# mprib/caliscope

Hardware: NVIDIA H100
Metric: lm_iterations_per_sec (higher is better)
Workload: dtype f64

## Files before the change

### caliscope_b200/csrc/cb_engine.cu

```cuda
#include <cuda_runtime.h>
#include <dlfcn.h>
#if defined(__x86_64__)
#include <emmintrin.h>
#endif
#include <nvtx3/nvToolsExt.h>

#include <algorithm>
#include <atomic>
#include <chrono>
#include <cmath>
#include <limits>
#include <cstdio>
#include <cstdlib>
#include <cstring>
#include <condition_variable>
#include <cub/cub.cuh>
#include <deque>
#include <functional>
#include <map>
#include <memory>
#include <mutex>
#include <string>
#include <thread>
#include <type_traits>
// ... 509 lines not shown
    k.trial_reduce = cb::trial_reduce_kernel<S>;
    k.schur_finalize = cb::schur_finalize_kernel<S>;
    k.schur_finalize_peer = cb::schur_finalize_peer_kernel<S>;
    with_bool(held.cams(), [&](auto hc) {
      constexpr bool HC = decltype(hc)::value;
      k.reduced_prep = cb::reduced_prep_kernel<S, HC>;
      k.small_rig_step = cb::small_rig_step_kernel<S, HC>;
    });
    k.comp_build = cb::comp_build_kernel<S>;
    k.cov_point = cb::cov_point_kernel<S>;
    with_lanes(pt_lanes, [&](auto lanes) {
      constexpr int L = decltype(lanes)::value;
      k.pt_stage_bytes = cb::pt_stage_bytes<S, L>();
      with_bool(cam_in_smem, [&](auto sm) {
        constexpr bool SM = decltype(sm)::value;
        with_bool(!held.fixp.empty(), [&](auto fp) {
          k.pt_backsub = cb::pt_backsub_kernel<S, L, SM, decltype(fp)::value>;
        });
        with_bool(held.points(), [&](auto hp) {
          constexpr bool HP = decltype(hp)::value;
          with_bool(dups, [&](auto d) {
            constexpr bool D = decltype(d)::value;
            k.pt_pass = cb::pt_pass_kernel<S, L, D, SM, false, HP>;
            k.pt_pass_cov = cb::pt_pass_kernel<S, L, D, SM, true, HP>;
          });
        });
      });
    });
    if (pcg_mode != 2) k.pcg = cb::pcg_cluster_kernel<1, S, 1>;
    else
      k.pcg = pcg_cl == 2 ? cb::pcg_cluster_kernel<2, S, 2> : pcg_cl == 6 ? cb::pcg_cluster_kernel<2, S, 6>
            : pcg_cl == 12 ? cb::pcg_cluster_kernel<2, S, 12> : cb::pcg_cluster_kernel<2, S, 18>;
  });
  return k;
}

struct CbBaProblem {
  int device = 0, num_sms = 132;
  int n_cams = 0, n_pts = 0, P = 6, nP = 0, n_obs = 0, n_params = 0;
  int LD = 0, n_blk = 0, n_tiles = 0, n_split = 1, k_chunks = 0, K_pad = 0;
  int n_chunks = 0, pt_grid = 0, pt_lanes = 32, n_dups = 0;
  int cam_in_smem = 0;
  size_t pt_smem = 0, bs_smem = 0;
  Kernels k;
  std::vector<int> h_cam_off;
  std::vector<int> h_perm, h_slot;
  std::vector<int> h_iflags;
  bool order_auto = false, order_identity = true;
  int ncp = 0;
  int *d_cam_xoff = nullptr, *d_cam_slot = nullptr, *d_klist = nullptr;
  bool schur_sparse = false;
  double schur_flop_issued = 0.0;
  std::vector<void*> allocs;
  int* d_cam_flags = nullptr;
  double* d_cam_const = nullptr;
  double2 *d_cm_xy = nullptr, *d_pm_xy = nullptr;
  int *d_cm_pt = nullptr, *d_cm_orig = nullptr, *d_cam_start = nullptr;
  int *d_chunk_cam = nullptr, *d_chunk_begin = nullptr, *d_chunk_end = nullptr, *d_cam_chunk_start = nullptr;
  int *d_pt_start = nullptr, *d_pm_orig = nullptr, *d_pm_cam = nullptr, *d_pm_pt = nullptr;
  const int *d_obs_cam = nullptr, *d_obs_pt = nullptr;
  const double* d_obs_xy = nullptr;
  std::vector<int> h_cam_flags;
  std::vector<double> h_cam_const;
  int *d_tile_of = nullptr, *d_tile_slot_start = nullptr, *d_tile_slots = nullptr;
  cb::SyItem* d_items = nullptr;
  int n_items = 0, n_slots = 0;
  CUtensorMap zt_map{};
  unsigned char* d_active = nullptr;
  HeldSet held;
  double *d_lo = nullptr, *d_hi = nullptr;
  int bounds_for = -1;
  double *d_x = nullptr, *d_xc[2] = {nullptr, nullptr}, *d_xp4[2] = {nullptr, nullptr};
  double *d_camtab[2] = {nullptr, nullptr}, *d_Upk[2] = {nullptr, nullptr}, *d_gc[2] = {nullptr, nullptr},
         *d_costsum[2] = {nullptr, nullptr};
  double *d_partial = nullptr, *d_camcost = nullptr, *d_V6 = nullptr, *d_gp = nullptr, *d_Dp2 = nullptr,
         *d_Dc2 = nullptr, *d_Linv6 = nullptr, *d_tvec = nullptr, *d_Zt = nullptr, *d_part = nullptr,
         *d_tpart = nullptr, *d_red = nullptr, *d_Minv = nullptr, *d_dc = nullptr, *d_dp = nullptr,
         *d_bpart = nullptr, *d_sc = nullptr, *d_red2 = nullptr, *d_out2 = nullptr;
  unsigned long long* d_gmax = nullptr;
  unsigned int* d_counter = nullptr;
  cb::LmState* d_state = nullptr;
  cb::LmState* h_state = nullptr;
  cb::LmLogRow* d_log = nullptr;
  int log_cap = 4096;
  cudaEvent_t ev0 = nullptr, ev1 = nullptr, ev2 = nullptr, ev3 = nullptr, ev_state[2] = {nullptr, nullptr};
  cudaEvent_t ev_pp[2][4] = {{nullptr, nullptr, nullptr, nullptr}, {nullptr, nullptr, nullptr, nullptr}};
  cudaStream_t cap_stream = nullptr;
  TrialGraph trial_graph;
  TrialGraph loop_graph;
  int pcg_cs = 1, pcg_rows = 0, pcg_mode = 2, pcg_cl = 1, pcg_npa = 0;
  bool direct_solve = false;
  size_t direct_smem = 0;
  size_t pcg_smem = 0;
  int n_c = 0, n_comp = 0, n_dim_max = 0, n_cblk = 0;
  cb::ConstraintTables ct = {};
  double *d_c_rs[2] = {nullptr, nullptr}, *d_c_dirw[2] = {nullptr, nullptr}, *d_compL = nullptr, *d_gpt = nullptr;
  int* d_pt_comp = nullptr;
  size_t comp_build_smem = 0, comp_back_smem = 0;
  std::vector<int> h_ga, h_gb;
  std::vector<double> h_cdist, h_cw;
  int red_slots = 64;
  CbPeerGroup* peer = nullptr;
  int cov_n = 0;
  double *d_covA = nullptr, *d_covC = nullptr, *d_covD = nullptr, *d_covS = nullptr, *d_covDiag = nullptr,
         *d_covR = nullptr, *d_covPt = nullptr;
  int *d_covRank = nullptr, *d_covFail = nullptr;
  unsigned char* d_covFree = nullptr;
  float cov_ms[3] = {0.f, 0.f, 0.f};
  double solve_host_us[4] = {0.0, 0.0, 0.0, 0.0};
  size_t red_len() const { return (size_t)nP * nP + 3 * (size_t)nP + 1 + red_slots; }
  cb::CPtr2 c_camtab() const { return {{d_camtab[0], d_camtab[1]}}; }
  cb::Ptr2 m_camtab() const { return {{d_camtab[0], d_camtab[1]}}; }
  cb::CPtr2 c_xp() const { return {{d_xp4[0], d_xp4[1]}}; }
  cb::Ptr2 m_xp() const { return {{d_xp4[0], d_xp4[1]}}; }
  cb::Ptr2 m_xc() const { return {{d_xc[0], d_xc[1]}}; }
  cb::CPtr2 c_Upk() const { return {{d_Upk[0], d_Upk[1]}}; }
  cb::Ptr2 m_Upk() const { return {{d_Upk[0], d_Upk[1]}}; }
  cb::CPtr2 c_gc() const { return {{d_gc[0], d_gc[1]}}; }
  cb::Ptr2 m_gc() const { return {{d_gc[0], d_gc[1]}}; }
  cb::CPtr2 c_costsum() const { return {{d_costsum[0], d_costsum[1]}}; }
  cb::Ptr2 m_costsum() const { return {{d_costsum[0], d_costsum[1]}}; }
  cb::CPtr2 c_crs() const { return {{d_c_rs[0], d_c_rs[1]}}; }
  cb::Ptr2 m_crs() const { return {{d_c_rs[0], d_c_rs[1]}}; }
  cb::CPtr2 c_cdirw() const { return {{d_c_dirw[0], d_c_dirw[1]}}; }
  cb::Ptr2 m_cdirw() const { return {{d_c_dirw[0], d_c_dirw[1]}}; }
};

namespace {

template <typename T>
int palloc(CbBaProblem* p, T** ptr, size_t n) {
  CB_TRY(dalloc(ptr, n));
  p->allocs.push_back((void*)*ptr);
  return CB_OK;
}

int bits_for(unsigned long long v) {
  int b = 1;
  while (b < 64 && (v >> b) != 0ull) ++b;
  return b;
}

void destroy_graph(TrialGraph& g) {
  if (g.exec) cudaGraphExecDestroy(g.exec);
  if (g.graph) cudaGraphDestroy(g.graph);
  g.exec = nullptr; g.graph = nullptr; g.valid = false; g.n_kernels = 0;
}

cudaStream_t side_stream() {
  thread_local std::map<int, cudaStream_t> streams;
  int dev = 0;
  cudaGetDevice(&dev);
  auto it = streams.find(dev);
  if (it != streams.end()) return it->second;
  cudaStream_t s = nullptr;
  cudaStreamCreateWithFlags(&s, cudaStreamNonBlocking);
  streams[dev] = s;
  return s;
}

int choose_camera_order(CbBaProblem* p, const int* cam_order, cudaStream_t st) {
  const int nc = p->n_cams;
  p->h_perm.resize(nc); p->h_slot.resize(nc);
  for (int i = 0; i < nc; ++i) p->h_perm[i] = i;
  p->order_auto = false;
  if (cam_order) {
    std::vector<char> seen(nc, 0);
    for (int i = 0; i < nc; ++i) {
      const int c = cam_order[i];
      if (c < 0 || c >= nc || seen[c]) { g_last_error = "cam_order is not a permutation of 0..n_cams-1"; return CB_E_INVALID; }
      seen[c] = 1;
      p->h_perm[i] = c;
    }
  } else {
    const int cams_per_tile = std::max(1, cb::SY_TILE / p->P);
    const double avg = (double)p->n_obs / std::max(p->n_pts, 1);
    if (p->n_blk >= 3 && avg <= nc / 3.0) {
      p->order_auto = true;
      const int stride = std::max(1, p->n_pts / 8192), ns = cdiv(p->n_pts, stride);
      unsigned int* d_W;
      ScopedFree sf(st);
      CB_TRY(sf.alloc(&d_W, (size_t)nc * nc));
      CB_CUDA(cudaMemsetAsync(d_W, 0, sizeof(unsigned int) * nc * nc, st));
      CB_LAUNCH(cb::covis_kernel, cdiv((long long)ns * 32, 256), 256, 0, st, p->d_pt_start, p->d_pm_cam, p->n_pts, stride, nc, d_W);
      std::vector<unsigned int> W((size_t)nc * nc);
      CB_CUDA(cudaMemcpyAsync(W.data(), d_W, sizeof(unsigned int) * nc * nc, cudaMemcpyDeviceToHost, st));
      CB_CUDA(cudaStreamSynchronize(st));
      std::vector<char> placed(nc, 0);
      std::vector<int> order;
      int start = 0;
      unsigned long long best = ~0ull;
      for (int c = 0; c < nc; ++c) {
        unsigned long long tot = 0;
        for (int q = 0; q < nc; ++q) if (q != c) tot += W[(size_t)c * nc + q];
        if (tot < best) { best = tot; start = c; }
      }
      order.push_back(start); placed[start] = 1;
      while ((int)order.size() < nc) {
        int pick = -1;
        unsigned long long bw = 0;
        const int lo = std::max(0, (int)order.size() - cams_per_tile);
        for (int c = 0; c < nc; ++c) {
          if (placed[c]) continue;
          unsigned long long w = 0;
          for (int k = lo; k < (int)order.size(); ++k) w += W[(size_t)c * nc + order[k]];
          if (pick < 0 || w > bw) { pick = c; bw = w; }
        }
        order.push_back(pick); placed[pick] = 1;
      }
      auto off_mass = [&](const std::vector<int>& ord) {
        std::vector<int> tile(nc);
        for (int i = 0; i < nc; ++i) tile[ord[i]] = (i * p->P) / cb::SY_TILE;
        unsigned long long m = 0;
        for (int a = 0; a < nc; ++a)
          for (int b = 0; b < nc; ++b)
            if (tile[a] != tile[b]) m += W[(size_t)a * nc + b];
        return m;
      };
      std::vector<int> ident(nc);
      for (int i = 0; i < nc; ++i) ident[i] = i;
      if (off_mass(order) < 0.8 * off_mass(ident)) p->h_perm = order;
    }
  }
  p->order_identity = true;
  for (int i = 0; i < nc; ++i) {
    p->h_slot[p->h_perm[i]] = i;
    if (p->h_perm[i] != i) p->order_identity = false;
  }
  CB_CUDA(cudaMemcpyAsync(p->d_cam_slot, p->h_slot.data(), sizeof(int) * nc, cudaMemcpyHostToDevice, st));
  return CB_OK;
}

struct XyUpload {
  bool started = false;
  std::atomic<int> finished{0};
  cudaEvent_t ev = nullptr;
  int rc = CB_OK;
  std::string err;
  ScopedFree pinned;
  void join() {
    if (!started) return;
    while (!finished.load(std::memory_order_acquire)) std::this_thread::yield();
    started = false;
  }
  int wait(cudaStream_t st) {
    join();
    if (rc != CB_OK) { g_last_error = err; return rc; }
    if (ev) CB_CUDA(cudaStreamWaitEvent(st, ev, 0));
    return CB_OK;
  }
  ~XyUpload() {
    join();
    if (ev) { cudaEventSynchronize(ev); cudaEventDestroy(ev); }
  }
};

int build_indices(CbBaProblem* p, const int* d_obs_cam, const int* d_obs_pt, const double* d_obs_xy,
                  const int* cam_order, cudaStream_t st, XyUpload* xy_upload) {
  const int n = p->n_obs;
  const int TB = 256, G = cdiv(std::max(n, 1), TB);
  ScopedFree sf(st);
  int* d_bad;
  CB_TRY(sf.alloc(&d_bad, 2));
  CB_CUDA(cudaMemsetAsync(d_bad, 0, 2 * sizeof(int), st));
  CB_LAUNCH(cb::validate_kernel, G, TB, 0, st, d_obs_cam, d_obs_pt, n, p->n_cams, p->n_pts, d_bad);

  unsigned long long *k_in, *k_out;
  int *v_in, *v_out, *pm_pt, *pm_cam, *cm_cam;
  CB_TRY(sf.alloc(&k_in, n));
  CB_TRY(sf.alloc(&k_out, n));
  CB_TRY(sf.alloc(&v_in, n));
  CB_TRY(sf.alloc(&v_out, n));
  CB_TRY(sf.alloc(&cm_cam, n));
  pm_pt = p->d_pm_pt; pm_cam = p->d_pm_cam;

  CB_LAUNCH(cb::make_keys_kernel, G, TB, 0, st, d_obs_pt, d_obs_cam, (long long)p->n_cams, n, k_in, v_in);
  const int kb = bits_for((unsigned long long)p->n_pts * (unsigned long long)p->n_cams);
  CB_CUB(sf, cub::DeviceRadixSort::SortPairs, k_in, k_out, v_in, p->d_pm_orig, n, 0, kb, st);
  g_launches.fetch_add(4);
  CB_LAUNCH(cb::split_keys_kernel, G, TB, 0, st, k_out, (long long)p->n_cams, n, pm_pt, pm_cam);
  CB_LAUNCH(cb::lower_bound_kernel, cdiv(p->n_pts + 1, TB), TB, 0, st, pm_pt, n, p->n_pts, p->d_pt_start);
  CB_LAUNCH(cb::count_dups_kernel, G, TB, 0, st, pm_pt, pm_cam, n, d_bad + 1);
  CB_TRY(choose_camera_order(p, cam_order, st));
  if (!p->order_identity) CB_LAUNCH(cb::remap_kernel, G, TB, 0, st, pm_cam, (const int*)p->d_cam_slot, n);
  CB_LAUNCH(cb::make_keys_kernel, G, TB, 0, st, pm_cam, pm_pt, (long long)p->n_pts, n, k_in, v_in);
  CB_CUB(sf, cub::DeviceRadixSort::SortPairs, k_in, k_out, v_in, v_out, n, 0, kb, st);
  g_launches.fetch_add(4);
  CB_LAUNCH(cb::split_keys_kernel, G, TB, 0, st, k_out, (long long)p->n_pts, n, cm_cam, v_in);
  CB_LAUNCH(cb::lower_bound_kernel, cdiv(p->n_cams + 1, TB), TB, 0, st, cm_cam, n, p->n_cams, p->d_cam_start);
  if (xy_upload) CB_TRY(xy_upload->wait(st));
  CB_LAUNCH(cb::cm_gather_kernel, G, TB, 0, st, v_out, p->d_pm_orig, pm_pt,
            reinterpret_cast<const double2*>(d_obs_xy), n, p->d_cm_pt, p->d_cm_orig, p->d_cm_xy);
  CB_LAUNCH(cb::pm_gather_kernel, G, TB, 0, st, p->d_pm_orig, reinterpret_cast<const double2*>(d_obs_xy), n, p->d_pm_xy);
  std::vector<int> cam_start(p->n_cams + 1);
  int bad[2] = {0, 0};
  CB_CUDA(cudaMemcpyAsync(cam_start.data(), p->d_cam_start, sizeof(int) * (p->n_cams + 1), cudaMemcpyDeviceToHost, st));
  CB_CUDA(cudaMemcpyAsync(bad, d_bad, 2 * sizeof(int), cudaMemcpyDeviceToHost, st));
  CB_CUDA(cudaStreamSynchronize(st));
  if (bad[0]) {
    g_last_error = "obs_cam / obs_pt index out of range in " + std::to_string(bad[0]) + " observations";
    return CB_E_INVALID;
  }
  p->n_dups = bad[1];
  std::vector<int> cc, cbeg, cend, ccs(p->n_cams + 1);
  const int chunk = cb::RJ_CHUNK;
  for (int c = 0; c < p->n_cams; ++c) {
    ccs[c] = (int)cc.size();
    for (int b = cam_start[c]; b < cam_start[c + 1]; b += chunk) {
      cc.push_back(c);
      cbeg.push_back(b);
      cend.push_back(std::min(b + chunk, cam_start[c + 1]));
    }
  }
  ccs[p->n_cams] = (int)cc.size();
  p->n_chunks = (int)cc.size();
  CB_TRY(palloc(p, &p->d_chunk_cam, cc.size()));
  CB_TRY(palloc(p, &p->d_chunk_begin, cc.size()));
  CB_TRY(palloc(p, &p->d_chunk_end, cc.size()));
  if (!cc.empty()) {
    CB_CUDA(cudaMemcpyAsync(p->d_chunk_cam, cc.data(), sizeof(int) * cc.size(), cudaMemcpyHostToDevice, st));
    CB_CUDA(cudaMemcpyAsync(p->d_chunk_begin, cbeg.data(), sizeof(int) * cc.size(), cudaMemcpyHostToDevice, st));
    CB_CUDA(cudaMemcpyAsync(p->d_chunk_end, cend.data(), sizeof(int) * cc.size(), cudaMemcpyHostToDevice, st));
  }
  CB_CUDA(cudaMemcpyAsync(p->d_cam_chunk_start, ccs.data(), sizeof(int) * ccs.size(), cudaMemcpyHostToDevice, st));
  CB_CUDA(cudaStreamSynchronize(st));
  return CB_OK;
}

int run_cam_prep(CbBaProblem* p, const double* xc, double* camtab, cudaStream_t st) {
  CB_LAUNCH(cb::cam_prep_kernel, cdiv(p->n_cams, 64), 64, 0, st, xc, p->d_cam_flags, p->d_cam_const, p->n_cams, p->P, camtab);
  return CB_OK;
}

void launch_resjac(CbBaProblem* p, int mode, const cb::LmState* st_dev, int flip, int loss, double fscale, double* out2,
                   cudaStream_t st) {
  if (p->n_chunks == 0) return;
  CB_LAUNCH(p->k.resjac[mode], p->n_chunks, cb::RJ_THREADS, 0, st, st_dev, flip, p->d_chunk_cam,
            p->d_chunk_begin, p->d_chunk_end, p->d_cm_xy, p->d_cm_pt, p->d_cm_orig, p->c_camtab(), p->c_xp(), loss,
            fscale, p->d_partial, out2);
}

void launch_pt_pass(CbBaProblem* p, bool cov, cudaStream_t st) {
  const auto pt_pass = cov ? p->k.pt_pass_cov : p->k.pt_pass;
  CB_LAUNCH(pt_pass, p->pt_grid, cb::PT_WARPS * 32, p->pt_smem, st, p->d_state,
            p->d_pt_start, p->d_pm_cam, p->d_pm_xy, p->d_pt_comp, p->n_pts, p->n_cams, p->c_camtab(), p->c_xp(),
            p->d_V6, p->d_gp, p->d_Dp2, cov ? p->d_covR : p->d_Linv6, p->d_tvec, p->d_Zt, (size_t)p->LD, p->d_gmax,
            cov ? p->d_covRank : nullptr, p->held.ppri);
}

void launch_pt_backsub(CbBaProblem* p, double* dp_out, cudaStream_t st) {
  const int bstride = p->pt_grid + p->n_comp;
  CB_LAUNCH(p->k.pt_backsub, p->pt_grid, cb::PT_WARPS * 32, p->bs_smem, st, p->d_state,
            p->d_pt_start, p->d_pm_cam, p->d_pm_xy, p->d_pt_comp, p->n_pts, p->n_cams, p->nP, p->c_camtab(),
            p->m_xp(), p->d_dc, p->d_Linv6, p->d_tvec, p->d_gp, p->d_Dp2, dp_out, p->d_bpart, bstride);
}

int launch_pcg(CbBaProblem* p, const cb::LmState* st_dev, double tol2, int max_iter, cudaStream_t st) {
  const ClusterConfig c(p->pcg_cs, cb::PCG_THREADS, p->pcg_cs, p->pcg_smem, st);
  const double* S = p->d_red;
  const double* b = p->d_red + (size_t)p->nP * p->nP;
  CB_CUDA(cudaLaunchKernelEx(&c.cfg, p->k.pcg, st_dev, S, b, (const double*)p->d_Minv, p->nP, p->pcg_npa, p->pcg_rows,
                             tol2, max_iter, p->d_dc, p->d_sc));
  g_launches.fetch_add(1);
  return CB_OK;
}

int camera_pass(CbBaProblem* p, int flip, int mode, cudaStream_t st) {
  const int loss = 0;
  const double fscale = 1.0;
  launch_resjac(p, 0, p->d_state, flip, loss, fscale, nullptr, st);
  if (p->n_c)
    CB_LAUNCH((cb::constraint_eval_kernel<false>), p->n_cblk, cb::CC_THREADS, 0, st, (const cb::LmState*)p->d_state, flip,
              p->ct, p->c_xp(), loss, fscale, p->m_crs(), p->m_cdirw(), (double*)nullptr, p->d_camcost + p->n_cams);
  const HeldSet& h = p->held;
  if (h.priors())
    CB_LAUNCH(cb::prior_cost_kernel, h.n_prior_blk, cb::PRIOR_THREADS, 0, st, (const cb::LmState*)p->d_state, flip, p->P,
              h.cpri, h.ppri, p->c_xp(), p->d_camcost + p->n_cams + p->n_cblk);
  CB_LAUNCH(p->k.trial_reduce, p->n_cams + 1, 64, 0, st, p->d_state, mode, p->n_cams, p->d_cam_chunk_start,
            p->d_partial, p->m_Upk(), p->m_gc(), p->m_costsum(), p->d_camcost, p->n_cblk + h.n_prior_blk, p->d_bpart,
            p->pt_grid + p->n_comp, p->pt_grid + p->n_comp, p->d_red2, p->d_counter, p->d_sc, p->d_log);
  return CB_OK;
}

int build_system(CbBaProblem* p, const CbBaOptions* opt, cudaStream_t st, const cudaEvent_t* ev = nullptr, bool cov = false) {
  if (ev) CB_CUDA(cudaEventRecord(ev[0], st));
  launch_pt_pass(p, cov, st);
  if (ev) CB_CUDA(cudaEventRecord(ev[1], st));
  if (p->n_c)
    CB_LAUNCH(p->k.comp_build, p->n_comp, cb::CC_THREADS, p->comp_build_smem, st, (const cb::LmState*)p->d_state,
              p->ct, p->d_pt_start, p->d_pm_cam, p->d_V6, p->d_gp, p->d_Dp2, p->d_gpt, p->c_crs(), p->c_cdirw(), p->n_cams,
              p->d_compL, p->d_tvec, p->d_Zt, (size_t)p->LD, p->d_gmax);
  if (ev) CB_CUDA(cudaEventRecord(ev[2], st));
  CB_LAUNCH(cb::schur_syrk_kernel, p->n_items, cb::SY_THREADS, sizeof(cb::SyrkSmem), st, p->zt_map,
            (const cb::LmState*)p->d_state, p->d_Zt, (size_t)p->LD, p->d_tvec, p->d_items, (const int*)p->d_klist,
            p->d_part, p->d_tpart);
  if (ev) CB_CUDA(cudaEventRecord(ev[3], st));
  const size_t nfin = (size_t)p->nP * p->nP + p->nP + 1;
  const int rank = sharded(opt) ? std::min(std::max(opt->rank, 0), p->red_slots - 1) : 0;
  if (opt && opt->peer_group) {
    CbPeerGroup* g = (CbPeerGroup*)opt->peer_group;
    int nb = 0;
    CB_CUDA(cudaOccupancyMaxActiveBlocksPerMultiprocessor(&nb, p->k.schur_finalize_peer, cb::PEER_THREADS, 0));
    const int grid = std::max(1, std::min(nb, 2)) * p->num_sms;
    const cb::LmState* sd = p->d_state;
    int nP = p->nP, n_blk = p->n_blk, red_slots = p->red_slots, rk = rank;
    cb::CPtr2 upk = p->c_Upk(), gc = p->c_gc(), cs = p->c_costsum();
    const double* gmax = (const double*)p->d_gmax;
    void* args[] = {&sd, &nP, &n_blk, &p->d_tile_of, &p->d_tile_slot_start, &p->d_tile_slots, &p->d_part, &p->d_tpart,
                    &upk, &gc, &cs, &gmax, &red_slots, &rk, &g->tab, &p->d_red};
    CB_CUDA(cudaLaunchCooperativeKernel((const void*)p->k.schur_finalize_peer, dim3(grid), dim3(cb::PEER_THREADS),
                                        args, 0, st));
    g_launches.fetch_add(1);
  } else {
    CB_LAUNCH(p->k.schur_finalize, cdiv((long long)std::max<size_t>(nfin, p->red_slots), 256), 256, 0, st,
              (const cb::LmState*)p->d_state, p->nP, p->n_blk, p->d_tile_of, p->d_tile_slot_start, p->d_tile_slots,
              p->d_part, p->d_tpart, p->c_Upk(), p->c_gc(), p->c_costsum(), (const double*)p->d_gmax, p->red_slots, rank,
              p->d_red);
    if (sharded(opt)) CB_TRY(do_allreduce(opt, p->d_red, (long long)p->red_len(), st));
  }
  if (!p->direct_solve && !cov)
    CB_LAUNCH(p->k.reduced_prep, 1, 256, 0, st, p->d_state, p->nP, p->n_cams, p->red_slots, p->d_red, p->d_Dc2,
              p->d_active, p->d_Minv, p->d_gmax, p->d_sc, (const int*)p->held.d_fixc, (int)p->held.fixc_x.size(),
              (const cb::CamPriors*)p->held.d_cpri);
  return CB_OK;
}

int solve_step(CbBaProblem* p, double* dp_out, cudaStream_t st) {
  const size_t nn = (size_t)p->nP * p->nP;
  if (p->direct_solve) {
    CB_LAUNCH(p->k.small_rig_step, 1, cb::DIRECT_THREADS, p->direct_smem, st, p->d_state, p->nP, p->n_cams,
              p->red_slots, p->d_red, p->d_Dc2, p->d_active, p->d_gmax, p->d_sc, p->m_xc(), p->d_dc, p->d_lo, p->d_hi,
              p->d_cam_flags, p->d_cam_const, p->m_camtab(), (const int*)p->held.d_fixc, (int)p->held.fixc_x.size(),
              (const cb::CamPriors*)p->held.d_cpri);
  } else {
    CB_TRY(launch_pcg(p, p->d_state, 0.0, 0, st));
    CB_LAUNCH(cb::cam_step_kernel, 1, 256, 0, st, (const cb::LmState*)p->d_state, p->nP, p->n_cams, p->P, p->m_xc(), p->d_dc,
              p->d_lo, p->d_hi, p->d_red + nn + p->nP, p->d_Dc2, p->d_active, p->d_cam_flags, p->d_cam_const, p->m_camtab(),
              p->d_sc);
  }
  launch_pt_backsub(p, dp_out, st);
  if (p->n_c)
    CB_LAUNCH(cb::comp_backsub_kernel, p->n_comp, cb::CC_THREADS, p->comp_back_smem, st, (const cb::LmState*)p->d_state,
              p->ct, p->nP, p->d_Zt, (size_t)p->LD, p->d_dc, p->d_compL, p->d_tvec, p->d_gpt, p->d_Dp2, p->m_xp(), dp_out,
              p->d_bpart, p->pt_grid + p->n_comp, p->pt_grid);
  return CB_OK;
}

int enqueue_trial(CbBaProblem* p, const CbBaOptions* opt, cudaStream_t st, const cudaEvent_t* ev = nullptr) {
  CB_TRY(build_system(p, opt, st, ev));
  CB_TRY(solve_step(p, nullptr, st));
  const bool multi = sharded(opt);
  CB_TRY(camera_pass(p, 1, multi ? 2 : 1, st));
  if (multi) {
    cb::PeerTable none = {};
    if (opt->peer_group) {
      CB_LAUNCH(cb::lm_decide_kernel, 1, 32, 0, st, p->d_state, (const double*)p->d_sc, p->d_red2, p->d_log,
                ((CbPeerGroup*)opt->peer_group)->tab, 1);
    } else {
      CB_TRY(do_allreduce(opt, p->d_red2, 4, st));
      CB_LAUNCH(cb::lm_decide_kernel, 1, 32, 0, st, p->d_state, (const double*)p->d_sc, p->d_red2, p->d_log, none, 0);
    }
  }
  return CB_OK;
}

int upload_x(CbBaProblem* p, const double* x, cudaStream_t st, bool fresh = false) {
  CB_CUDA(cudaMemcpyAsync(p->d_x, x, sizeof(double) * p->n_params, cudaMemcpyHostToDevice, st));
  const int n = std::max(std::max(p->n_cams * p->P, p->n_pts), fresh ? (int)cb::SC_COUNT : 1);
  const cb::FreshState z = fresh ? cb::FreshState{p->d_gmax, p->d_counter, p->d_sc, p->d_Dc2, p->d_Dp2} : cb::FreshState{};
  CB_LAUNCH(cb::unpack_x_kernel, cdiv(n, 256), 256, 0, st, p->d_x, p->d_cam_xoff, p->d_cam_flags, p->d_cam_const,
            p->n_cams, p->P, p->n_pts, p->ncp, p->d_xc[0], p->d_xp4[0], z);
  const std::vector<int>& fixp = p->held.fixp;
  if (!fixp.empty())
    CB_LAUNCH(cb::mark_fixed_points_kernel, cdiv((int)fixp.size(), 256), 256, 0, st, (const int*)p->held.d_fixp,
              (int)fixp.size(), p->d_xp4[0]);
  return CB_OK;
}

int download_x(CbBaProblem* p, double* x, cudaStream_t st) {
  const int n = std::max(p->n_cams * p->P, p->n_pts);
  CB_LAUNCH(cb::pack_x_kernel, cdiv(std::max(n, 1), 256), 256, 0, st, p->d_x, p->d_cam_xoff, p->d_cam_flags, p->n_cams,
            p->P, p->n_pts, p->ncp, (const cb::LmState*)p->d_state, cb::CPtr2{{p->d_xc[0], p->d_xc[1]}}, p->c_xp());
  CB_CUDA(cudaMemcpyAsync(x, p->d_x, sizeof(double) * p->n_params, cudaMemcpyDeviceToHost, st));
  return CB_OK;
}

int set_bounds(CbBaProblem* p, bool use_bounds, cudaStream_t st) {
  if (p->bounds_for == (use_bounds ? 1 : 0)) return CB_OK;
  std::vector<double> lo((size_t)p->nP, -1e300), hi((size_t)p->nP, 1e300);
  if (use_bounds && p->P == 9) {
    for (int c = 0; c < p->n_cams; ++c)
      if (p->h_iflags[c] & CB_CAM_FREE_INTRINSICS) {
        lo[c * 9 + 6] = 0.5; hi[c * 9 + 6] = 2.0;
        lo[c * 9 + 7] = -1.0; hi[c * 9 + 7] = 1.0;
        lo[c * 9 + 8] = -2.0; hi[c * 9 + 8] = 2.0;
      }
  }
  CB_CUDA(cudaMemcpyAsync(p->d_lo, lo.data(), sizeof(double) * p->nP, cudaMemcpyHostToDevice, st));
  CB_CUDA(cudaMemcpyAsync(p->d_hi, hi.data(), sizeof(double) * p->nP, cudaMemcpyHostToDevice, st));
  p->bounds_for = use_bounds ? 1 : 0;
  return CB_OK;
}

int init_state(CbBaProblem* p, const CbBaOptions* opt, double lam, long long max_nfev, cudaStream_t st) {
  cb::LmState& h = p->h_state[3];
  std::memset(&h, 0, sizeof(h));
  h.lam = lam; h.nu = 2.0;
  h.ftol = opt->ftol; h.xtol = opt->xtol; h.gtol = opt->gtol;
  h.nfev = 1; h.njev = 1; h.nit = 0; h.max_nfev = max_nfev;
  h.new_lin = 1;
  h.log_cap = p->log_cap;
  h.loss = opt->loss;
  h.fscale = opt->f_scale > 0 ? opt->f_scale : 1.0;
  const double tol = opt->pcg_tol > 0 ? opt->pcg_tol : 1e-6;
  h.pcg_tol2 = tol * tol;
  h.pcg_max_iter = opt->pcg_max_iter > 0 ? opt->pcg_max_iter : 4 * p->nP;
  if (opt->peer_group) {
    CbPeerGroup* g = (CbPeerGroup*)opt->peer_group;
    h.epoch_big = g->epoch_big; h.epoch_small = g->epoch_small;
  }
  CB_CUDA(cudaMemcpyAsync(p->d_state, &h, sizeof(h), cudaMemcpyHostToDevice, st));
  return CB_OK;
}

int ensure_graph(CbBaProblem* p, const CbBaOptions* opt, bool loop) {
  TrialGraph& g = loop ? p->loop_graph : p->trial_graph;
  const TrialGraph::Key key{opt->nccl_comm, opt->peer_group, opt->rank, opt->world_size};
  if (g.key == key && (g.valid || g.failed)) return g.valid ? CB_OK : CB_E_UNSUPPORTED;
  destroy_graph(g);
  g.key = key;
  g.failed = false;
  auto fail = [&](const char* what) {
    g_last_error = std::string(loop ? "device-loop graph: " : "trial graph: ") + what + ": " +
                   cudaGetErrorString(cudaGetLastError());
    destroy_graph(g);
    g.failed = true;
    return CB_E_UNSUPPORTED;
  };
  if (!p->cap_stream && cudaStreamCreateWithFlags(&p->cap_stream, cudaStreamNonBlocking) != cudaSuccess)
    return fail("cudaStreamCreateWithFlags");
  cudaGraphConditionalHandle h = {};
  cudaError_t e;
  if (loop) {
    if (cudaGraphCreate(&g.graph, 0) != cudaSuccess) return fail("cudaGraphCreate");
    if (cudaGraphConditionalHandleCreate(&h, g.graph, 1, cudaGraphCondAssignDefault) != cudaSuccess)
      return fail("cudaGraphConditionalHandleCreate");
    cudaGraphNodeParams np = {};
    np.type = cudaGraphNodeTypeConditional;
    np.conditional.handle = h;
    np.conditional.type = cudaGraphCondTypeWhile;
    np.conditional.size = 1;
    cudaGraphNode_t node;
    if (cudaGraphAddNode(&node, g.graph, nullptr, 0, &np) != cudaSuccess) return fail("cudaGraphAddNode(conditional)");
    e = cudaStreamBeginCaptureToGraph(p->cap_stream, np.conditional.phGraph_out[0], nullptr, nullptr, 0,
                                      cudaStreamCaptureModeThreadLocal);
  } else {
    e = cudaStreamBeginCapture(p->cap_stream, cudaStreamCaptureModeThreadLocal);
  }
  if (e != cudaSuccess) return fail("begin capture");
  const long long l0 = g_launches.load();
  int rc = enqueue_trial(p, opt, p->cap_stream);
  if (loop && rc == CB_OK) CB_LAUNCH(cb::lm_loop_cond_kernel, 1, 1, 0, p->cap_stream, (const cb::LmState*)p->d_state, h);
  g.n_kernels = (int)(g_launches.load() - l0);
  g_launches.store(l0);
  e = loop ? cudaStreamEndCapture(p->cap_stream, nullptr) : cudaStreamEndCapture(p->cap_stream, &g.graph);
  if (rc != CB_OK || e != cudaSuccess) return fail("capture of the trial");
  if (cudaGraphInstantiate(&g.exec, g.graph, 0) != cudaSuccess) return fail("cudaGraphInstantiate");
  g.valid = true;
  return CB_OK;
}

int lm_solve(CbBaProblem* p, const CbBaOptions* opt, const double* x0, double* x_out, CbBaResult* res, cudaStream_t st) {
  NvtxRange nvtx_solve("cb_ba_solve");
  const long long max_nfev = opt->max_nfev > 0 ? opt->max_nfev : 100ll * p->n_params;
  const bool verbose = opt->verbose >= 2 && opt->rank == 0;
  const long long launches0 = g_launches.load();
  std::memset(res, 0, sizeof(*res));

  const bool direct = opt->allreduce != nullptr || opt->time_kernels;
  bool use_loop = !direct && !sharded(opt);
  if (use_loop && ensure_graph(p, opt, true) != CB_OK) { cudaGetLastError(); use_loop = false; }
  bool use_graph = !direct && !use_loop;
  if (use_graph && ensure_graph(p, opt, false) != CB_OK) { cudaGetLastError(); use_graph = false; }

  auto t_mark = std::chrono::steady_clock::now();
  auto host_span = [&](int i) {
    const auto now = std::chrono::steady_clock::now();
    p->solve_host_us[i] = std::chrono::duration<double, std::micro>(now - t_mark).count();
    t_mark = now;
  };
  CB_TRY(set_bounds(p, opt->use_bounds != 0, st));
  host_span(0);
  CB_TRY(init_state(p, opt, opt->lambda0 > 0 ? opt->lambda0 : 1e-4, max_nfev, st));
  host_span(1);
  CB_TRY(upload_x(p, x0, st, true));
  host_span(2);
  CB_CUDA(cudaEventRecord(p->ev0, st));
  CB_TRY(run_cam_prep(p, p->d_xc[0], p->d_camtab[0], st));
  CB_TRY(camera_pass(p, 0, 0, st));

  double pp_ms_total = 0.0;
  long long pp_launches = 0, trials = 0;
  double sy_ms_total = 0.0;
  long long sy_launches = 0;
  auto read_pp = [&](long long t) {
    float ms = 0.f;
    const cudaEvent_t* ev = p->ev_pp[t & 1];
    if (cudaEventElapsedTime(&ms, ev[0], ev[1]) == cudaSuccess) { pp_ms_total += ms; ++pp_launches; }
    else cudaGetLastError();
    if (cudaEventElapsedTime(&ms, ev[2], ev[3]) == cudaSuccess) { sy_ms_total += ms; ++sy_launches; }
    else cudaGetLastError();
  };
  bool done = false;
  long long t = 0;
// ... 4335 lines not shown
```

### caliscope_b200/csrc/cb_kernels.cuh

```cuda
#pragma once
#include <cooperative_groups.h>

#include "cb_device.cuh"

namespace cb {
namespace cg = cooperative_groups;

constexpr int RJ_THREADS = 128;
constexpr int RJ_CHUNK = 2048;
constexpr int PT_WARPS = 8;
constexpr int SY_TILE = 96;
constexpr int SY_KC = 32;
constexpr int SY_STAGES = 4;
constexpr int SY_CONSUMER_WARPS = 8;
constexpr int SY_THREADS = 32 * (SY_CONSUMER_WARPS + 1);
constexpr int PCG_THREADS = 512;

template <int P>
struct RowT {
  static constexpr int NU = P * (P + 1) / 2;
  static constexpr int NACC = NU + P + 1;
};

enum {
  SC_COST = 0, SC_GNORM_C, SC_COST_NEW, SC_PRED_C, SC_STEP2_C, SC_X2_C, SC_PRED_P, SC_STEP2_P, SC_X2_P,
  SC_PCG_ITS, SC_PCG_REL, SC_PCG_FLAG, SC_GNORM_P, SC_PCG_T0 = 16, SC_COUNT = 24
};

struct FreshState {
  unsigned long long* gmax;
  unsigned int* counter;
  double *sc, *Dc2, *Dp2;
};

__global__ void unpack_x_kernel(const double* __restrict__ x, const int* __restrict__ cam_xoff,
                                const int* __restrict__ cam_flags, const double* __restrict__ cam_const,
                                int n_cams, int P, int n_pts, int ncp, double* __restrict__ xc, double* __restrict__ xp4,
                                FreshState z) {
  int i = blockIdx.x * blockDim.x + threadIdx.x;
  if (z.Dp2 != nullptr) {
    if (i < 2) z.gmax[i] = 0ull;
    if (i < 4) z.counter[i] = 0u;
    if (i < SC_COUNT) z.sc[i] = 0.0;
    if (i < n_cams * P) z.Dc2[i] = 0.0;
    if (i < n_pts) { z.Dp2[3 * (size_t)i] = 0.0; z.Dp2[3 * (size_t)i + 1] = 0.0; z.Dp2[3 * (size_t)i + 2] = 0.0; }
  }
  if (i < n_cams * P) {
    int c = i / P, p = i % P;
    int w = (cam_flags[c] & 1) ? 9 : 6;
    double v;
    if (p < w) v = x[cam_xoff[c] + p];
    else v = (p == 6) ? 1.0 : cam_const[c * 9 + 4 + (p - 7)];
    xc[i] = v;
  }
  if (i < n_pts) {
    xp4[4 * (size_t)i + 0] = x[ncp + 3 * (size_t)i + 0];
    xp4[4 * (size_t)i + 1] = x[ncp + 3 * (size_t)i + 1];
    xp4[4 * (size_t)i + 2] = x[ncp + 3 * (size_t)i + 2];
    xp4[4 * (size_t)i + 3] = 0.0;
  }
}

__global__ void mark_fixed_points_kernel(const int* __restrict__ pts, int n, double* __restrict__ xp4) {
  const int i = blockIdx.x * blockDim.x + threadIdx.x;
  if (i < n) xp4[4 * (size_t)pts[i] + 3] = 1.0;
}

struct LmState {
  double lam, nu, cost, gnorm, initial_cost;
  double ftol, xtol, gtol;
  long long nfev, njev, nit, max_nfev, pcg_total;
  unsigned long long epoch_big, epoch_small;
  double fscale, pcg_tol2;
  int cur, done, status, new_lin, err, bad_streak, n_log, log_cap;
  int loss, pcg_max_iter;
};
struct Ptr2 {
  double* p[2];
};
struct CPtr2 {
  const double* p[2];
};

__global__ void pack_x_kernel(double* __restrict__ x, const int* __restrict__ cam_xoff, const int* __restrict__ cam_flags,
                              int n_cams, int P, int n_pts, int ncp, const LmState* __restrict__ st, CPtr2 xc2, CPtr2 xp2) {
  const bool sel = st->cur != 0;
  const double* __restrict__ xc = sel ? xc2.p[1] : xc2.p[0];
  const double* __restrict__ xp4 = sel ? xp2.p[1] : xp2.p[0];
  int i = blockIdx.x * blockDim.x + threadIdx.x;
  if (i < n_cams * P) {
    int c = i / P, p = i % P;
    if (p < ((cam_flags[c] & 1) ? 9 : 6)) x[cam_xoff[c] + p] = xc[i];
  }
  if (i < n_pts) {
    x[ncp + 3 * (size_t)i + 0] = xp4[4 * (size_t)i + 0];
    x[ncp + 3 * (size_t)i + 1] = xp4[4 * (size_t)i + 1];
    x[ncp + 3 * (size_t)i + 2] = xp4[4 * (size_t)i + 2];
  }
}

__device__ __forceinline__ void cam_prep_rot(double r0, double r1, double r2, double* __restrict__ o) {
  const double th2 = r0 * r0 + r1 * r1 + r2 * r2, th = sqrt(th2);
  double R[9];
  double s = 0.0, co = 1.0;
  if (th >= 1e-12) sincos(th, &s, &co);
  if (th < 1e-12) {
    R[0] = 1; R[1] = -r2; R[2] = r1; R[3] = r2; R[4] = 1; R[5] = -r0; R[6] = -r1; R[7] = r0; R[8] = 1;
  } else {
    const double it = 1.0 / th, kx = r0 * it, ky = r1 * it, kz = r2 * it, c1 = 1.0 - co;
    R[0] = co + c1 * kx * kx;      R[1] = c1 * kx * ky - s * kz; R[2] = c1 * kx * kz + s * ky;
    R[3] = c1 * ky * kx + s * kz;  R[4] = co + c1 * ky * ky;     R[5] = c1 * ky * kz - s * kx;
    R[6] = c1 * kz * kx - s * ky;  R[7] = c1 * kz * ky + s * kx; R[8] = co + c1 * kz * kz;
  }
  double B, C;
  if (th < 1e-4) {
    B = 0.5 - th2 / 24.0 + th2 * th2 / 720.0;
    C = 1.0 / 6.0 - th2 / 120.0 + th2 * th2 / 5040.0;
  } else {
    B = (1.0 - co) / th2;
    C = (th - s) / (th2 * th);
  }
  const double K2[9] = {r0 * r0 - th2, r0 * r1, r0 * r2, r1 * r0, r1 * r1 - th2, r1 * r2, r2 * r0, r2 * r1, r2 * r2 - th2};
  const double Km[9] = {0, -r2, r1, r2, 0, -r0, -r1, r0, 0};
#pragma unroll
  for (int i = 0; i < 9; ++i) {
    o[CT_R + i] = R[i];
    o[CT_JR + i] = ((i % 4 == 0) ? 1.0 : 0.0) - B * Km[i] + C * K2[i];
  }
}

__device__ __forceinline__ void cam_prep_one(const double* __restrict__ q, const double* __restrict__ k, int flags,
                                             double* __restrict__ o) {
  const bool free_i = (flags & 1) != 0;
  cam_prep_rot(q[0], q[1], q[2], o);
  o[CT_T + 0] = q[3]; o[CT_T + 1] = q[4]; o[CT_T + 2] = q[5];
  double sc = 1.0, k1 = k[4], k2 = k[5];
  if (free_i) { sc = q[6]; k1 = q[7]; k2 = q[8]; }
  const double fx = sc * k[0], fy = sc * k[1];
  o[CT_FX] = fx; o[CT_FY] = fy; o[CT_CX] = k[2]; o[CT_CY] = k[3];
  o[CT_D + 0] = k1; o[CT_D + 1] = k2; o[CT_D + 2] = k[6]; o[CT_D + 3] = k[7]; o[CT_D + 4] = k[8];
  o[CT_IFX0] = 1.0 / k[0];
  o[CT_SX] = fx / k[0];
  o[CT_SY] = fy / k[0];
  o[CT_FYR] = k[1] / k[0];
  o[CT_FLAGS] = (double)flags;
  o[CT_FX0] = k[0];
}

__global__ void cam_prep_kernel(const double* __restrict__ xc, const int* __restrict__ cam_flags,
                                const double* __restrict__ cam_const, int n_cams, int P,
                                double* __restrict__ camtab) {
  int c = blockIdx.x * blockDim.x + threadIdx.x;
  if (c >= n_cams) return;
  cam_prep_one(xc + (size_t)c * P, cam_const + (size_t)c * 9, cam_flags[c], camtab + (size_t)c * CT_SIZE);
}

template <int P, int MODE>
__global__ void __launch_bounds__(RJ_THREADS, (MODE == 0 && P == 6) ? 3 : 1)
resjac_kernel(const LmState* __restrict__ st, int flip, const int* __restrict__ chunk_cam,
              const int* __restrict__ chunk_begin, const int* __restrict__ chunk_end,
              const double2* __restrict__ cm_xy, const int* __restrict__ cm_pt, const int* __restrict__ cm_orig,
              CPtr2 camtab2, CPtr2 xp2, int loss, double fscale, double* __restrict__ partial,
              double* __restrict__ out2) {
  using RT = RowT<P>;
  __shared__ double cam[CT_SIZE];
  __shared__ double red[(MODE == 0 ? RT::NACC : 1) * (RJ_THREADS / 32)];
  int sel = 0;
  if (st != nullptr) {
    if (st->done) return;
    sel = st->cur ^ flip;
    loss = st->loss;
    fscale = st->fscale;
  }
  const double* __restrict__ camtab = camtab2.p[sel];
  const double* __restrict__ xp4 = xp2.p[sel];
  const int chunk = blockIdx.x;
  const int c = chunk_cam[chunk];
  const int begin = chunk_begin[chunk], end = chunk_end[chunk];
  if (threadIdx.x < CT_SIZE) cam[threadIdx.x] = camtab[(size_t)c * CT_SIZE + threadIdx.x];
  __syncthreads();
  const int flags = (int)cam[CT_FLAGS];
  const bool fish = (flags & 2) != 0;

  double acc[(MODE == 0) ? RT::NACC : 1];
#pragma unroll
  for (int k = 0; k < ((MODE == 0) ? RT::NACC : 1); ++k) acc[k] = 0.0;

  int q = begin + threadIdx.x;
  double2 xy_a = make_double2(0.0, 0.0), xy_b = xy_a;
  int pt_a = 0, org_a = 0, pt_b = 0, org_b = 0;
  double Xn0 = 0.0, Xn1 = 0.0, Xn2 = 0.0, Xn3 = 0.0;
  auto load_idx = [&](int qq, double2& xy, int& pt, int& org) {
    if (qq < end) {
      xy = cm_xy[qq];
      pt = cm_pt[qq];
      if constexpr (MODE == 2 || MODE == 3) org = cm_orig[qq];
    }
  };
  load_idx(q, xy_a, pt_a, org_a);
  load_idx(q + RJ_THREADS, xy_b, pt_b, org_b);
  if (q < end) ld256nc(xp4 + 4 * (size_t)pt_a, Xn0, Xn1, Xn2, Xn3);
  for (; q < end; q += RJ_THREADS) {
    const double2 xy = xy_a;
    const int org = org_a;
    const double X0 = Xn0, X1 = Xn1, X2 = Xn2;
    (void)org;
    xy_a = xy_b; pt_a = pt_b; org_a = org_b;
    if (q + RJ_THREADS < end) ld256nc(xp4 + 4 * (size_t)pt_a, Xn0, Xn1, Xn2, Xn3);
    load_idx(q + 2 * RJ_THREADS, xy_b, pt_b, org_b);
    if constexpr (MODE == 0) {
      double f[2], JX[6], Jc[2 * P];
      acc[RT::NACC - 1] += obs_jac<P>(cam, X0, X1, X2, xy.x, xy.y, loss, fscale, f, JX, Jc);
      int u = 0;
#pragma unroll
      for (int a = 0; a < P; ++a)
#pragma unroll
        for (int b = a; b < P; ++b) {
          acc[u] = fma(Jc[a], Jc[b], fma(Jc[P + a], Jc[P + b], acc[u]));
          ++u;
        }
#pragma unroll
      for (int a = 0; a < P; ++a) acc[RT::NU + a] = fma(Jc[a], f[0], fma(Jc[P + a], f[1], acc[RT::NU + a]));
    } else {
      ProjOut o;
      project_obs<false>(cam, fish, X0, X1, X2, o);
      const double ex = o.u - xy.x, ey = o.v - xy.y;
      if constexpr (MODE == 3) {
        const size_t i = (size_t)org;
        out2[2 * i] = ex; out2[2 * i + 1] = ey;
      } else if constexpr (MODE == 4) {
        out2[q] = sqrt(__dadd_rn(__dmul_rn(ex, ex), __dmul_rn(ey, ey)));
      } else {
        const double f0 = ex * cam[CT_IFX0], f1 = ey * cam[CT_IFX0];
        if constexpr (MODE == 2) {
          const size_t i = (size_t)org;
          out2[2 * i] = f0; out2[2 * i + 1] = f1;
        } else {
          acc[0] += robust_cost_only(loss, fscale, f0) + robust_cost_only(loss, fscale, f1);
        }
      }
    }
  }
  if constexpr (MODE == 0 || MODE == 1) {
    constexpr int NA = (MODE == 0) ? RT::NACC : 1;
    const int lane = threadIdx.x & 31, wid = threadIdx.x >> 5;
#pragma unroll
    for (int k = 0; k < NA; ++k) {
      double v = warp_sum(acc[k]);
      if (lane == 0) red[wid * NA + k] = v;
    }
    __syncthreads();
    if (threadIdx.x < NA) {
      double v = 0.0;
#pragma unroll
      for (int w = 0; w < RJ_THREADS / 32; ++w) v += red[w * NA + threadIdx.x];
      partial[(size_t)chunk * NA + threadIdx.x] = v;
    }
  }
}

__global__ void sum_kernel(const double* __restrict__ in, int n, double* __restrict__ out) {
  __shared__ double sh[32];
  double v = 0.0;
  for (int i = threadIdx.x; i < n; i += blockDim.x) v += in[i];
  v = warp_sum(v);
  if ((threadIdx.x & 31) == 0) sh[threadIdx.x >> 5] = v;
  __syncthreads();
  if (threadIdx.x < 32) {
    v = (threadIdx.x < (blockDim.x >> 5)) ? sh[threadIdx.x] : 0.0;
    v = warp_sum(v);
    if (threadIdx.x == 0) out[0] = v;
  }
}

template <int P>
__global__ void jac_blocks_kernel(const int* __restrict__ obs_cam, const int* __restrict__ cam_slot,
                                  const int* __restrict__ obs_pt,
                                  const double2* __restrict__ obs_xy, int n, const double* __restrict__ camtab,
                                  const double* __restrict__ xp4, double* __restrict__ Jc_out,
                                  double* __restrict__ Jp_out) {
  const int i = blockIdx.x * blockDim.x + threadIdx.x;
  if (i >= n) return;
  const double* X = xp4 + 4 * (size_t)obs_pt[i];
  const double2 xy = obs_xy[i];
  double f[2], JX[6], Jc[2 * P];
  obs_jac<P>(camtab + (size_t)cam_slot[obs_cam[i]] * CT_SIZE, X[0], X[1], X[2], xy.x, xy.y, 0, 1.0, f, JX, Jc);
  for (int k = 0; k < 6; ++k) Jp_out[(size_t)i * 6 + k] = JX[k];
  for (int r = 0; r < 2; ++r)
    for (int p = 0; p < 9; ++p) Jc_out[(size_t)i * 18 + r * 9 + p] = (p < P) ? Jc[r * P + p] : 0.0;
}

__device__ __forceinline__ void chol3_inv(const double* V6, const double* D2, double lam, double* Li) {
  const double d0 = D2[0] > 0.0 ? D2[0] : 1.0, d1 = D2[1] > 0.0 ? D2[1] : 1.0, d2 = D2[2] > 0.0 ? D2[2] : 1.0;
  const double e00 = V6[0] + lam * d0, e01 = V6[1], e02 = V6[2], e11 = V6[3] + lam * d1, e12 = V6[4],
               e22 = V6[5] + lam * d2;
  bool ok = e00 > 0.0;
  const double i00 = rsqrt(ok ? e00 : 1.0);
  const double l10 = e01 * i00, l20 = e02 * i00;
  const double t11 = e11 - l10 * l10;
  ok = ok && t11 > 0.0;
  const double i11 = rsqrt(ok ? t11 : 1.0);
  const double l21 = (e12 - l20 * l10) * i11;
  const double t22 = e22 - l20 * l20 - l21 * l21;
  ok = ok && t22 > 0.0;
  const double i22 = rsqrt(ok ? t22 : 1.0);
  const double i10 = -l10 * i00 * i11;
  const double i21 = -l21 * i11 * i22;
  const double i20 = -(l20 * i00 + l21 * i10) * i22;
  if (ok) {
    Li[0] = i00; Li[1] = i10; Li[2] = i11; Li[3] = i20; Li[4] = i21; Li[5] = i22;
  } else {
    Li[0] = Li[1] = Li[2] = Li[3] = Li[4] = Li[5] = 0.0;
// ... 853 lines not shown
```

Measured before the change: 925.7.

## Size resjac chunks from occupancy to balance waves across SMs

Replaces the fixed 2048-observation per-camera chunking with a host-side search. It picks the number of chunks per camera so the total fits a whole number of waves, using occupancy times SM count as the slot count. The cost model weighs wave count against the longest chunk length plus a fixed per-chunk overhead. The goal is to remove tail imbalance and idle SMs in the residual/Jacobian kernel, at the price of more setup work on the host and possibly more per-chunk reduction overhead. A profiling script for SASS-based FP64 and HBM floor estimates is also added.

New measurement: 901.5 (median of 6 runs). 2.6% lower.

```diff
diff --git a/caliscope_b200/csrc/cb_engine.cu b/caliscope_b200/csrc/cb_engine.cu
--- a/caliscope_b200/csrc/cb_engine.cu
+++ b/caliscope_b200/csrc/cb_engine.cu
@@ -835,14 +835,43 @@
     return CB_E_INVALID;
   }
   p->n_dups = bad[1];
+  int rj_blocks = 0;
+  CB_CUDA(cudaOccupancyMaxActiveBlocksPerMultiprocessor(
+      &rj_blocks, p->P == 9 ? cb::resjac_kernel<9, 0> : cb::resjac_kernel<6, 0>, cb::RJ_THREADS, 0));
+  const long long slots = (long long)std::max(rj_blocks, 1) * p->num_sms;
+  std::vector<int> pieces(p->n_cams, 0);
+  {
+    int seen = 0;
+    for (int c = 0; c < p->n_cams; ++c) seen += cam_start[c + 1] > cam_start[c];
+    long long best_cost = -1;
+    for (int w = 1; w <= std::max(8, cdiv(seen, slots)); ++w) {
+      const long long cap = w * slots;
+      if (cap < seen) continue;
+      long long len = std::max<long long>(cb::RJ_MIN_CHUNK, cdiv(p->n_obs, cap));
+      std::vector<int> pc(p->n_cams);
+      for (;; len += std::max<long long>(1, len / 64)) {
+        long long total = 0;
+        for (int c = 0; c < p->n_cams; ++c) {
+          pc[c] = cdiv(cam_start[c + 1] - cam_start[c], len);
+          total += pc[c];
+        }
+        if (total <= cap) break;
+      }
+      long long longest = 0;
+      for (int c = 0; c < p->n_cams; ++c)
+        if (pc[c]) longest = std::max<long long>(longest, cdiv(cam_start[c + 1] - cam_start[c], pc[c]));
+      const long long cost = w * (cdiv(longest, cb::RJ_THREADS) + cb::RJ_CHUNK_COST);
+      if (best_cost < 0 || cost < best_cost) { best_cost = cost; pieces = pc; }
+    }
+  }
   std::vector<int> cc, cbeg, cend, ccs(p->n_cams + 1);
-  const int chunk = cb::RJ_CHUNK;
   for (int c = 0; c < p->n_cams; ++c) {
     ccs[c] = (int)cc.size();
-    for (int b = cam_start[c]; b < cam_start[c + 1]; b += chunk) {
+    const int n_c = cam_start[c + 1] - cam_start[c];
+    for (int k = 0; k < pieces[c]; ++k) {
       cc.push_back(c);
-      cbeg.push_back(b);
-      cend.push_back(std::min(b + chunk, cam_start[c + 1]));
+      cbeg.push_back(cam_start[c] + (int)((long long)n_c * k / pieces[c]));
+      cend.push_back(cam_start[c] + (int)((long long)n_c * (k + 1) / pieces[c]));
     }
   }
   ccs[p->n_cams] = (int)cc.size();
diff --git a/caliscope_b200/csrc/cb_kernels.cuh b/caliscope_b200/csrc/cb_kernels.cuh
--- a/caliscope_b200/csrc/cb_kernels.cuh
+++ b/caliscope_b200/csrc/cb_kernels.cuh
@@ -7,7 +7,8 @@
 namespace cg = cooperative_groups;
 
 constexpr int RJ_THREADS = 128;
-constexpr int RJ_CHUNK = 2048;
+constexpr int RJ_MIN_CHUNK = 512;
+constexpr int RJ_CHUNK_COST = 4;
 constexpr int PT_WARPS = 8;
 constexpr int SY_TILE = 96;
 constexpr int SY_KC = 32;
diff --git a/profiles/trial_tail_floors.py b/profiles/trial_tail_floors.py
--- /dev/null
+++ b/profiles/trial_tail_floors.py
@@ -0,0 +1,189 @@
+import argparse
+import json
+import re
+import subprocess
+import sys
+from pathlib import Path
+
+ROOT = Path(__file__).resolve().parent.parent
+sys.path.insert(0, str(ROOT))
+
+FP64 = ("DFMA", "DMUL", "DADD", "DSETP", "DMNMX")
+CLASSES = FP64 + ("MUFU", "SHFL", "LDG", "LDS", "STG")
+HBM_TBS = 3.35
+
+KERNELS = {
+    "cb::resjac_kernel<6, 0>": (24, "chunk"),
+    "cb::resjac_kernel<9, 0>": (24, "chunk"),
+    "cb::pt_backsub_kernel<6, 8, true, false>": (20, "point"),
+    "cb::pt_backsub_kernel<9, 8, true, false>": (20, "point"),
+}
+RJ_WAVE, RJ_THREADS, BS_LANES = {6: 396, 9: 264}, 128, 8
+
+INS = re.compile(r"^\s*/\*([0-9a-f]{4,})\*/\s+(@!?U?P[T0-9]+\s+)?([A-Z][A-Z0-9_.]*)(.*?);")
+LABEL = re.compile(r"^\s*(\.L_x_\d+):")
+TARGET = re.compile(r"`\((\.L_x_\d+)\)|\b(0x[0-9a-f]+)\b")
+
+
+def functions(lib: str) -> dict[str, list[str]]:
+    out = subprocess.run(["cuobjdump", "-sass", lib], capture_output=True, text=True, check=True).stdout
+    funcs, cur = {}, None
+    for line in out.splitlines():
+        m = re.match(r"^\s*Function : (\S+)", line)
+        if m:
+            cur = m.group(1)
+            funcs[cur] = []
+        elif cur is not None:
+            funcs[cur].append(line)
+    names = subprocess.run(["cu++filt"], input="\n".join(funcs), capture_output=True, text=True, check=True).stdout
+
+    def key(dm: str) -> str:
+        dm = re.sub(r"^void ", "", dm).replace("(int)", "").replace("(bool)1", "true").replace("(bool)0", "false")
+        return dm.split("(")[0]
+
+    return {key(dm): funcs[mg] for mg, dm in zip(funcs, names.splitlines())}
+
+
+def parse(lines: list[str]):
+    ins, labels, pending = [], {}, []
+    for line in lines:
+        m = LABEL.match(line)
+        if m:
+            pending.append(m.group(1))
+            continue
+        m = INS.match(line)
+        if m:
+            a = int(m.group(1), 16)
+            for lab in pending:
+                labels[lab] = a
+            pending = []
+            ins.append((a, (m.group(2) or "").strip(), m.group(3), m.group(4)))
+    return ins, labels
+
+
+def branch_target(ops: str, labels: dict) -> int | None:
+    m = TARGET.search(ops)
+    if not m:
+        return None
+    return labels[m.group(1)] if m.group(1) else int(m.group(2), 16)
+
+
+def classify(op: str) -> str | None:
+    base = op.split(".")[0]
+    return base if base in CLASSES else None
+
+
+def count(ins) -> dict:
+    c = {k: 0 for k in CLASSES}
+    for _, _, op, _ in ins:
+        k = classify(op)
+        if k:
+            c[k] += 1
+    return c
+
+
+def observation_loop(ins, labels):
+    idx = {a: i for i, (a, _, _, _) in enumerate(ins)}
+    loops = []
+    for i, (a, _, op, ops) in enumerate(ins):
+        if op.startswith("BRA"):
+            t = branch_target(ops, labels)
+            if t is not None and t <= a:
+                loops.append((idx[t], i))
+    inner = [lp for lp in loops if not any(o != lp and lp[0] <= o[0] and o[1] <= lp[1] for o in loops)]
+    fp = lambda lp: sum(1 for _, _, op, _ in ins[lp[0]:lp[1] + 1] if classify(op) in FP64)
+    return max(inner, key=fp)
+
+
+def cheapest_iteration(ins, labels, first: int, last: int) -> list:
+    idx = {a: i for i, (a, _, _, _) in enumerate(ins)}
+    lead = {first}
+    for i in range(first, last + 1):
+        _, _, op, ops = ins[i]
+        if op.startswith(("BRA", "EXIT", "RET", "BRX", "JMX")):
+            if i + 1 <= last:
+                lead.add(i + 1)
+            t = branch_target(ops, labels) if op.startswith("BRA") else None
+            if t is not None and first <= idx.get(t, -1) <= last:
+                lead.add(idx[t])
+    starts = sorted(lead)
+    blocks = {s: (s, (starts[k + 1] - 1) if k + 1 < len(starts) else last) for k, s in enumerate(starts)}
+    weight = lambda b: (sum(1 for _, _, op, _ in ins[b[0]:b[1] + 1] if classify(op) in FP64), b[1] - b[0] + 1)
+    INF = (1 << 30, 1 << 30)
+    best = {s: (INF, None) for s in starts}
+    best[first] = (weight(blocks[first]), None)
+    done_cost, done_at = INF, None
+    for s in starts:
+        cost, _ = best[s]
+        if cost == INF:
+            continue
+        _, b1 = blocks[s]
+        _, pred, op, ops = ins[b1]
+        succ = []
+        if op.startswith("BRA"):
+            t = branch_target(ops, labels)
+            if b1 == last:
+                if cost < done_cost:
+                    done_cost, done_at = cost, s
+            else:
+                if t is not None and first <= idx.get(t, -1) <= last:
+                    succ.append(idx[t])
+                if pred:
+                    succ.append(b1 + 1)
+        elif op.startswith(("EXIT", "RET", "BRX", "JMX")):
+            if pred:
+                succ.append(b1 + 1)
+        elif b1 + 1 <= last:
+            succ.append(b1 + 1)
+        for n in succ:
+            if n in blocks and n > s:
+                w = weight(blocks[n])
+                c = (cost[0] + w[0], cost[1] + w[1])
+                if c < best[n][0]:
+                    best[n] = (c, s)
+    path, s = [], done_at
+    while s is not None:
+        path.append(s)
+        s = best[s][1]
+    return [x for s in reversed(path) for x in ins[blocks[s][0]:blocks[s][1] + 1]]
+
+
+def main() -> None:
+    import bench
+
+    ap = argparse.ArgumentParser()
+    ap.add_argument("--lib", default=str(ROOT / "caliscope_b200" / "libcaliscope_b200.so"))
+    ap.add_argument("--workload", nargs="*", default=["cfg4", "cfg4_shard8"])
+    ap.add_argument("--dfma-tflops", type=float, default=33.0)
+    args = ap.parse_args()
+    funcs = functions(args.lib)
+    dfma_per_s = args.dfma_tflops * 1e12 / 2
+    for kname, (bytes_per_obs, share) in KERNELS.items():
+        if kname not in funcs:
+            print(json.dumps({"kernel": kname, "error": "not in the library"}))
+            continue
+        ins, labels = parse(funcs[kname])
+        first, last = observation_loop(ins, labels)
+        loop = count(cheapest_iteration(ins, labels, first, last))
+        once = count(ins[:first] + ins[last + 1:])
+        for w in args.workload:
+            n_c, n_p, n_o, _ = bench.WORKLOADS[w]
+            if share == "chunk":
+                per_obs = RJ_WAVE[9 if "<9" in kname else 6] * RJ_THREADS / n_o
+            else:
+                per_obs = n_p * BS_LANES / n_o
+            fp_loop = sum(loop[k] for k in FP64)
+            fp_once = sum(once[k] for k in FP64) * per_obs
+            fp64_us = n_o * fp_loop / dfma_per_s * 1e6
+            hbm_us = n_o * bytes_per_obs / (HBM_TBS * 1e12) * 1e6
+            print(json.dumps({
+                "kernel": kname, "workload": w, "n_obs": n_o,
+                "loop_per_obs": loop, "once_per_obs": {k: round(v * per_obs, 3) for k, v in once.items()},
+                "fp64_per_obs": fp_loop, "fp64_floor_us": round(fp64_us, 2),
+                "fp64_with_once_us": round(n_o * (fp_loop + fp_once) / dfma_per_s * 1e6, 2),
+                "hbm_floor_us": round(hbm_us, 2), "bound": "fp64" if fp64_us >= hbm_us else "hbm",
+            }))
+
+
+if __name__ == "__main__":
+    main()
```
